# faustomorales/keras-ocr

Measured on AMD Instinct MI355X. Metric: images/sec end-to-end Pipeline.recognize() @768x768, higher is better.
Workload: dtype f32 (fp32 operands as 2 fp16 pieces [F(4,3) / head layers] or 3 bf16 pieces [1x1, dilated], 3 / 6 MFMA products, fp32 accumulate; fp32-class error vs fp64: tests/test_conv_gpu.py)

## Files before the change

### include/kocr.h

```cpp
#ifndef KOCR_H
#define KOCR_H

#include <stdint.h>

#ifdef __cplusplus
extern "C" {
#endif

typedef struct kocr_ctx kocr_ctx;

enum {
  KOCR_OK = 0,
  KOCR_EINVAL = -1,
  KOCR_EHIP = -2,
  KOCR_ENOWEIGHTS = -3,
  KOCR_ECAPACITY = -4,
  KOCR_ENOMEM = -5,
  KOCR_EEMPTYCONTOUR = -6,
  KOCR_EZERODIV = -7
};

enum { KOCR_U8 = 0, KOCR_F32 = 1 };

int kocr_create(kocr_ctx** out, int hip_device);
// ... 71 lines not shown
                     int64_t cap_lines, int64_t* true_lines, int flags);

int kocr_detect(kocr_ctx* ctx, const void* img, int dtype, int N, int H, int W,
                float detection_threshold, float text_threshold, float link_threshold,
                int size_threshold, int micro_batch, float* boxes, int32_t* counts, int cap,
                int on_device);

int kocr_recognize_boxes(kocr_ctx* ctx, const uint8_t* img_rgb, int N, int H, int W,
                         const float* boxes, const int32_t* counts, int32_t* labels, int on_device);

int kocr_resize_pad(kocr_ctx* ctx, const uint8_t* src, int n, int sh, int sw, int dh, int dw,
                    int Hmax, int Wmax, int cval, uint8_t* dst, int on_device);

int kocr_pipeline(kocr_ctx* ctx, int N, const uint8_t* const* imgs, const int32_t* hs,
                  const int32_t* ws, const int32_t* dhs, const int32_t* dws, int Hmax, int Wmax,
                  float detection_threshold, float text_threshold, float link_threshold,
                  int size_threshold, int micro_batch, float* boxes, int32_t* counts, int cap,
                  int32_t* labels, int max_crops, int32_t* n_crops, int on_device);

int kocr_pipeline_results(kocr_ctx* ctx, float* boxes, int cap, int32_t* labels, int max_crops);

int kocr_pipeline_device_results(kocr_ctx* ctx, const float** d_boxes, const int32_t** d_counts, const int32_t** d_labels,
                                 int32_t* N, int32_t* cap, int32_t* M);

int kocr_conv2d_nhwc(kocr_ctx* ctx, const float* in, int N, int H, int W, int Cin,
                     const float* w_hwio, int KH, int KW, int dilation, int Cout,
                     const float* pre_a, const float* pre_b, int relu,
                     const float* post_a, const float* post_b, float* out);

int kocr_conv2d_cells(kocr_ctx* ctx, const float* in, int N, int H, int W, int Cin, const float* w_hwio, int Cout,
                      const float* pre_a, const float* pre_b, int relu, const float* post_a, const float* post_b,
                      int cellW, int cellWv, int pool, float* out, float* pool_out, float* amax_out);

#define KOCR_SPLIT_BF16X3 0
#define KOCR_SPLIT_F16X2 1
#define KOCR_SPLIT_F16X1 2
int kocr_set_split_mode(kocr_ctx* ctx, int mode);
int kocr_get_split_mode(const kocr_ctx* ctx);

int kocr_set_schedule(kocr_ctx* ctx, int fold_linear_chain, int fold_upsample);
int kocr_get_schedule(kocr_ctx* ctx, int* fold_linear_chain, int* fold_upsample);

#define KOCR_RECT_EXACT 0
#define KOCR_RECT_OPENCV 1
int kocr_set_min_area_rect(kocr_ctx* ctx, int rule);
int kocr_get_min_area_rect(const kocr_ctx* ctx);

int kocr_set_scores(kocr_ctx* ctx, int on);
int kocr_get_scores(const kocr_ctx* ctx);
int kocr_detection_scores(kocr_ctx* ctx, float* scores, int cap);
int kocr_recognition_scores(kocr_ctx* ctx, float* log_word, float* char_scores, int max_crops, int32_t* n_crops,
                            int32_t* label_width);
int kocr_crnn_forward_scores(kocr_ctx* ctx, const float* crops, int M, int32_t* labels, float* probs, float* log_word,
                             float* char_scores, int on_device);

int kocr_crnn_beam(kocr_ctx* ctx, const float* crops, int M, int beam_width, int top_paths, int32_t* labels, float* log_prob,
                   int on_device);
int kocr_set_beam(kocr_ctx* ctx, int beam_width, int top_paths);
int kocr_get_beam(const kocr_ctx* ctx, int* beam_width, int* top_paths);
int kocr_recognition_beams(kocr_ctx* ctx, int32_t* labels, float* log_prob, int max_crops, int32_t* n_crops,
                           int32_t* label_width, int32_t* top_paths);

#define KOCR_LEXICON_MAX_WORD 32
int kocr_set_lexicon(kocr_ctx* ctx, const int32_t* words, int stride, const int32_t* lengths, int V);
int kocr_lexicon_size(const kocr_ctx* ctx);
int kocr_crnn_lexicon(kocr_ctx* ctx, const float* crops, int M, int top_words, int32_t* index, float* log_prob, float* all_values,
// ... 19 lines not shown
```

### keras_ocr_amd/_lib.py

```python
import contextlib
import ctypes
import math
import os

import numpy as np

_HERE = os.path.dirname(os.path.abspath(__file__))
LIB_PATH = os.path.join(_HERE, "csrc", "libkocr.so")

KOCR_U8, KOCR_F32 = 0, 1
KOCR_OK, KOCR_EINVAL, KOCR_EHIP, KOCR_ENOWEIGHTS, KOCR_ECAPACITY, KOCR_ENOMEM, KOCR_EEMPTYCONTOUR, KOCR_EZERODIV = range(0, -8, -1)
MIN_AREA_RECT_RULES = {"exact": 0, "opencv": 1}

_c_float_p = ctypes.POINTER(ctypes.c_float)
_c_int_p = ctypes.POINTER(ctypes.c_int)
_c_i64_p = ctypes.POINTER(ctypes.c_int64)
_c_dbl_p = ctypes.POINTER(ctypes.c_double)

_lib = None


class KocrError(RuntimeError):
    """A libkocr call returned a non-zero code."""

# ... 46 lines not shown
        "kocr_set_lexicon_scratch": (ci, [vp, ctypes.c_uint64]),
        "kocr_set_scores": (ci, [vp, ci]),
        "kocr_get_scores": (ci, [vp]),
        "kocr_detection_scores": (ci, [vp, vp, ci]),
        "kocr_recognition_scores": (ci, [vp, vp, vp, ci, vp, vp]),
        "kocr_crnn_classes": (ci, [vp]),
        "kocr_crnn_label_width": (ci, [vp]),
        "kocr_crnn_set_rnn_steps_to_discard": (ci, [vp, ci]),
        "kocr_ctc_batch_cost": (ci, [vp, vp, ci, ci, ci, vp, ci, vp, vp, vp, ci]),
        "kocr_crnn_ctc_loss": (ci, [vp, vp, ci, vp, ci, vp, vp, vp, ci]),
        "kocr_crnn_features": (ci, [vp, vp, ci, vp, ci]),
        "kocr_compute_maps": (ci, [vp, vp, ci, ci, ci, ci, ci, ci, vp, vp, ci, vp, vp, vp, ci]),
        "kocr_heat_mse": (ci, [vp, vp, vp, ci, ci, ci, vp, ci]),
        "kocr_craft_mse": (ci, [vp, vp, ci, ci, ci, ci, vp, ci, vp, ci]),
        "kocr_iou_table": (ci, [vp, ci, vp, vp, vp, vp, vp, ctypes.c_int64, vp, ci]),
        "kocr_score": (ci, [vp, ci, vp, vp, vp, vp, vp, vp, vp, vp, vp, ctypes.c_double, ctypes.c_double, vp, vp, vp, vp, vp,
                            ctypes.c_int64, vp, ci]),
        "kocr_group_lines": (ci, [vp, ci, vp, vp, ctypes.c_double, ctypes.c_double, ctypes.c_double, ctypes.c_double, vp, vp, vp, vp,
                                  ctypes.c_int64, vp, ci]),
        "kocr_get_boxes": (ci, [vp, vp, ci, ci, ci, ctypes.c_float, ctypes.c_float, ctypes.c_float, ci, vp, vp, ci, ci]),
        "kocr_warp_crops": (ci, [vp, vp, ci, ci, ci, vp, vp, ci, ci, vp, ci]),
        "kocr_warp_quads": (ci, [vp, vp, ci, ci, ci, ci, vp, vp, vp, vp, vp, ci, ci, vp, vp]),
        "kocr_detect": (ci, [vp, vp, ci, ci, ci, ci, ctypes.c_float, ctypes.c_float, ctypes.c_float, ci, ci, vp, vp, ci, ci]),
        "kocr_recognize_boxes": (ci, [vp, vp, ci, ci, ci, vp, vp, vp, ci]),
        "kocr_resize_pad": (ci, [vp, vp, ci, ci, ci, ci, ci, ci, ci, ci, vp, ci]),
        "kocr_pipeline": (ci, [vp, ci, ctypes.POINTER(vp), _c_int_p, _c_int_p, _c_int_p, _c_int_p, ci, ci,
                               ctypes.c_float, ctypes.c_float, ctypes.c_float, ci, ci, vp, vp, ci, vp, ci, vp, ci]),
        "kocr_pipeline_device_results": (ci, [vp, vp, vp, vp, vp, vp, vp]),
        "kocr_pipeline_results": (ci, [vp, vp, ci, vp, ci]),
        "kocr_resize_pad_f32": (ci, [vp, vp, ci, ci, ci, ci, ci, ci, ci, ci, ctypes.c_float, vp]),
        "kocr_warp_crops_f32": (ci, [vp, vp, ci, ci, ci, ci, vp, vp, ci, ci, vp]),
        "kocr_conv2d_nhwc": (ci, [vp, vp, ci, ci, ci, ci, vp, ci, ci, ci, ci, vp, vp, ci, vp, vp, vp]),
        "kocr_conv2d_cells": (ci, [vp, vp, ci, ci, ci, ci, vp, ci, vp, vp, ci, vp, vp, ci, ci, ci, vp, vp, vp]),
        "kocr_set_split_mode": (ci, [vp, ci]),
        "kocr_get_split_mode": (ci, [vp]),
        "kocr_set_schedule": (ci, [vp, ci, ci]),
        "kocr_get_schedule": (ci, [vp, _c_int_p, _c_int_p]),
        "kocr_set_min_area_rect": (ci, [vp, ci]),
        "kocr_get_min_area_rect": (ci, [vp]),
        "kocr_profile_enable": (ci, [vp, ci]),
        "kocr_profile_reset": (ci, [vp]),
        "kocr_profile_report": (ci, [vp, ci, ctypes.c_char_p, _c_i64_p, _c_dbl_p, _c_dbl_p, _c_dbl_p]),
        "kocr_range_stats_enable": (ci, [vp, ci]),
        "kocr_range_stats_report": (ci, [vp, ci, ctypes.c_char_p, _c_dbl_p]),
    }
    for name, (res, args) in sigs.items():
        if not hasattr(lib, name):
            continue
        fn = getattr(lib, name)
        fn.restype = res
        fn.argtypes = args
    _lib = lib
    return lib


def _ptr(a):
    if a is None:
        return ctypes.c_void_p(0)
    if isinstance(a, (int, np.integer)):
        return ctypes.c_void_p(int(a))
    return ctypes.c_void_p(a.ctypes.data)


def beam_args(beam_width, top_paths=1):
    bw, k = int(beam_width), int(top_paths)
    if not 1 <= bw <= 64:
# ... 534 lines not shown
        self._check(self._lib.kocr_pipeline_device_results(self._h, ctypes.byref(pb), ctypes.byref(pc), ctypes.byref(pl),
                                                           ctypes.byref(n), ctypes.byref(cap), ctypes.byref(m)))
        return {"boxes": pb.value or 0, "counts": pc.value or 0, "labels": pl.value or 0, "n": n.value, "cap": cap.value, "m": m.value}

    def conv2d_nhwc(self, x, w_hwio, dilation=1, pre_a=None, pre_b=None, relu=False, post_a=None, post_b=None):
        x = np.ascontiguousarray(x, dtype=np.float32)
        w = np.ascontiguousarray(w_hwio, dtype=np.float32)
        n, h, wd, cin = x.shape
        kh, kw, cin2, cout = w.shape
        assert cin == cin2
        out = np.empty((n, h, wd, cout), dtype=np.float32)
        vecs = [None if v is None else np.ascontiguousarray(v, dtype=np.float32) for v in (pre_a, pre_b, post_a, post_b)]
        self._check(self._lib.kocr_conv2d_nhwc(self._h, _ptr(x), n, h, wd, cin, _ptr(w), kh, kw, int(dilation), cout,
                                               _ptr(vecs[0]), _ptr(vecs[1]), int(bool(relu)), _ptr(vecs[2]),
                                               _ptr(vecs[3]), _ptr(out)))
        return out

    def conv2d_cells(self, x, w_hwio, cell_w, cell_wv, pool=False, need_full=True, pre_a=None, pre_b=None, relu=False,
                     post_a=None, post_b=None):
        x = np.ascontiguousarray(x, dtype=np.float32)
        w = np.ascontiguousarray(w_hwio, dtype=np.float32)
        n, h, wd, cin = x.shape
        assert w.shape[:3] == (3, 3, cin)
        cout = w.shape[3]
        out = np.empty((n, h, wd, cout), dtype=np.float32) if (need_full or not pool) else None
        pooled = np.empty((n, h // 2, wd // 2, cout), dtype=np.float32) if pool else None
        amax = np.zeros((n, wd // cell_w), dtype=np.float32)
        vecs = [None if v is None else np.ascontiguousarray(v, dtype=np.float32) for v in (pre_a, pre_b, post_a, post_b)]
        self._check(self._lib.kocr_conv2d_cells(self._h, _ptr(x), n, h, wd, cin, _ptr(w), cout, _ptr(vecs[0]), _ptr(vecs[1]),
                                                int(bool(relu)), _ptr(vecs[2]), _ptr(vecs[3]), int(cell_w), int(cell_wv),
                                                int(bool(pool)), _ptr(out), _ptr(pooled), _ptr(amax)))
        return out, pooled, amax

    SPLIT_BF16X3, SPLIT_F16X2, SPLIT_F16X1 = 0, 1, 2

    def set_split_mode(self, mode):
        if isinstance(mode, str):
            mode = {"bf16": 0, "bf16x3": 0, "f16": 1, "fp16": 1, "f16x2": 1, "f16x1": 2, "fast": 2}[mode]
        self._check(self._lib.kocr_set_split_mode(self._h, int(mode)))

    def get_split_mode(self):
        return self._check(self._lib.kocr_get_split_mode(self._h))

    def set_schedule(self, fold_linear_chain=True, fold_upsample=True):
        self._check(self._lib.kocr_set_schedule(self._h, int(bool(fold_linear_chain)), int(bool(fold_upsample))))

    def get_schedule(self):
        lin, up = ctypes.c_int(0), ctypes.c_int(0)
        self._check(self._lib.kocr_get_schedule(self._h, ctypes.byref(lin), ctypes.byref(up)))
        return bool(lin.value), bool(up.value)

    def set_min_area_rect(self, rule):
        self._check(self._lib.kocr_set_min_area_rect(self._h, _min_area_rect_code(rule)))

    def get_min_area_rect(self):
        code = self._check(self._lib.kocr_get_min_area_rect(self._h))
        return {v: k for k, v in MIN_AREA_RECT_RULES.items()}[code]

    @contextlib.contextmanager
    def _min_area_rect_scope(self, rule):
        if rule is None:
            yield
            return
        code = _min_area_rect_code(rule)
        old = self._check(self._lib.kocr_get_min_area_rect(self._h))
        self._check(self._lib.kocr_set_min_area_rect(self._h, code))
# ... 191 lines not shown
```

### keras_ocr_amd/csrc/api.cpp

```cpp
#include "abi.h"
#include "taps.h"
#include <cmath>
#include <algorithm>
#include <mutex>
#include <set>

int arena_reserve(kocr_ctx* ctx, Arena& a, size_t bytes) {
  ctx->last_pl.valid = false;
  ctx->last_sc.clear();
  ctx->last_beam.clear();
  ctx->last_lex.clear();
  if (bytes <= a.cap) return KOCR_OK;
  if (a.base) {
    KOCR_HIP(ctx, hipStreamSynchronize(ctx->stream));
    KOCR_HIP(ctx, hipFree(a.base));
    a.base = nullptr;
    a.cap = 0;
  }
  const size_t want = bytes + (bytes >> 3) + 4096;
  void* p = nullptr;
  hipError_t e = hipMalloc(&p, want);
  if (e != hipSuccess) {
    ctx->set_err("workspace hipMalloc(" + std::to_string(want) + " B) failed: " + hipGetErrorString(e));
    return KOCR_ENOMEM;
// ... 912 lines not shown
  ti.C = ti.cs = Cin;
  to.C = to.cs = tp.C = tp.cs = Cout;
  ti.cellW = to.cellW = cellW;
  ti.cellWv = to.cellWv = cellWv;
  tp.cellW = cellW / 2;
  tp.cellWv = cellWv / 2;
  ti.amax = ctx->amax_slots(N * cn);
  to.amax = ctx->amax_slots(N * cn);
  tp.amax = ctx->amax_slots(N * cn);
  if (!ti.amax || !to.amax || !tp.amax) KOCR_FAIL(ctx, KOCR_ECAPACITY, "kocr_conv2d_cells: out of max-|x| slots");
  const float* d_in;
  KOCR_TRY(st.in(in, nin, d_in));
  ti.p = (float*)d_in;
  if (out) KOCR_TRY(st.out(out, nout, to.p));
  if (pool) KOCR_TRY(st.out(pool_out, npool, tp.p));
  std::vector<float> am((size_t)N * cn, 0.f);
  for (int n = 0; n < N; ++n)
    for (int y = 0; y < H; ++y)
      for (int x = 0; x < W; ++x) {
        const float* px = in + (((size_t)n * H + y) * W + x) * Cin;
        float m = 0.f;
        for (int c = 0; c < Cin; ++c) m = std::max(m, std::fabs(px[c]));
        float& a = am[(size_t)n * cn + x / cellW];
        a = std::max(a, m);
      }
  KOCR_TRY(st.put((float*)ti.amax, am.data(), am.size() * sizeof(float)));
  KOCR_TRY(launch_conv_pool(ctx, L, ti, nullptr, nullptr, to, pool ? &tp : nullptr, out != nullptr));
  if (out) KOCR_TRY(st.back(out, to.p, nout));
  if (pool) KOCR_TRY(st.back(pool_out, tp.p, npool));
  if (amax_out) KOCR_TRY(st.download(amax_out, (const float*)(pool && !out ? tp.amax : to.amax), am.size() * sizeof(float)));
  return st.finish();
}

int kocr_set_split_mode(kocr_ctx* ctx, int mode) {
  if (!ctx) return KOCR_EINVAL;
  if (mode != KOCR_SPLIT_BF16X3 && mode != KOCR_SPLIT_F16X2 && mode != KOCR_SPLIT_F16X1) KOCR_FAIL(ctx, KOCR_EINVAL, "kocr_set_split_mode: unknown mode");
  ctx->split_mode = mode;
  return KOCR_OK;
}

int kocr_get_split_mode(const kocr_ctx* ctx) { return ctx ? ctx->split_mode : KOCR_EINVAL; }

int kocr_set_schedule(kocr_ctx* ctx, int fold_linear_chain, int fold_upsample) {
  if (!ctx) return KOCR_EINVAL;
  ctx->opt_linfold = fold_linear_chain != 0;
  ctx->opt_upfold = fold_upsample != 0;
  return KOCR_OK;
}

int kocr_get_schedule(kocr_ctx* ctx, int* fold_linear_chain, int* fold_upsample) {
  if (!ctx || !fold_linear_chain || !fold_upsample) return KOCR_EINVAL;
  *fold_linear_chain = ctx->opt_linfold ? 1 : 0;
  *fold_upsample = ctx->opt_upfold ? 1 : 0;
  return KOCR_OK;
}

int kocr_set_min_area_rect(kocr_ctx* ctx, int rule) {
  if (!ctx) return KOCR_EINVAL;
  if (rule != KOCR_RECT_EXACT && rule != KOCR_RECT_OPENCV) KOCR_FAIL(ctx, KOCR_EINVAL, "kocr_set_min_area_rect: unknown rule");
  ctx->min_area_rect = rule;
  return KOCR_OK;
}

int kocr_get_min_area_rect(const kocr_ctx* ctx) { return ctx ? ctx->min_area_rect : KOCR_EINVAL; }

int kocr_set_scores(kocr_ctx* ctx, int on) {
// ... 103 lines not shown
```

### keras_ocr_amd/csrc/conv_w43h.hip

```cpp
#include "w43_common.h"
#include "probe_clock.h"

namespace {

#define W4H_SCALED_CONSTANTS(sc)                                                                       \
  const float k_s = (sc), k_sA = (sc) * W4_A, k_sB = (sc) * W4_B, k_sA2 = (sc) * W4_A2, k_sB2 = (sc) * W4_B2, \
              k_sA2B2 = (sc) * W4_A2B2, k_sA2PB2 = (sc) * W4_A2PB2
template <class T>
__device__ __forceinline__ T w4h_transform(const T (&d)[6], int xi, float k_s, float k_sA, float k_sB, float k_sA2, float k_sB2,
                                           float k_sA2B2, float k_sA2PB2) {
  switch (xi) {
    case 0: return (k_sA2B2 * d[0] - k_sA2PB2 * d[2]) + k_s * d[4];
    case 1: return (k_s * d[4] - k_sB2 * d[2]) + k_sA * (d[3] - W4_B2 * d[1]);
    case 2: return (k_s * d[4] - k_sB2 * d[2]) - k_sA * (d[3] - W4_B2 * d[1]);
    case 3: return (k_s * d[4] - k_sA2 * d[2]) + k_sB * (d[3] - W4_A2 * d[1]);
    case 4: return (k_s * d[4] - k_sA2 * d[2]) - k_sB * (d[3] - W4_A2 * d[1]);
    default: return (k_sA2B2 * d[1] - k_sA2PB2 * d[3]) + k_s * d[5];
  }
}

constexpr int W4H_TOP = 12;

}

// ... 219 lines not shown
  const unsigned wlane = (unsigned)lane * 16u;
  auto w_tile = [&](int nt) { return (unsigned)__builtin_amdgcn_readfirstlane((nt * 4 + wn) * 12 * 64 * 16); };
  hf8 bw[2][6][NP];
  f16v acc[6][2];
  const int a_lane = GEO == 2 ? slot(l31 >> 3, l5, l31 & 7) : slot(l31 >> 4, l5, l31 & 15);
  const int a_lane1 = GEO == 2 ? slot((l31 >> 3) + 1, l5, l31 & 7) : 0;
  auto load_a = [&](hf8 (&a)[2][NP], const unsigned short* bufp, int ky, int xi) __attribute__((always_inline)) {
    if constexpr (DBG & 8) return;
    const unsigned short* plane = bufp + xi * NP * PLANE_R;
#pragma unroll
    for (int s = NP - 1; s >= 0; --s)
#pragma unroll
      for (int m = 0; m < 2; ++m) {
        int off;
        if constexpr (GEO == 2) {
          const int c = ky + 4 * m;
          off = ((c & 1) ? a_lane1 : a_lane) + (c >> 1) * 256;
        } else {
          off = a_lane + (ky + 2 * m) * ROW_STRIDE;
        }
        a[m][s] = *reinterpret_cast<const hf8*>(plane + s * PLANE_R + off);
      }
  };
  auto mfma_pt = [&](const hf8 (&a)[2][NP], const hf8 (&b)[NP], int xi) __attribute__((always_inline)) {
    if constexpr (DBG & 4) {
#pragma unroll
      for (int m = 0; m < 2; ++m)
#pragma unroll
        for (int s = 0; s < NP; ++s) acc[xi][m][s] += __builtin_bit_cast(v4f, a[m][s])[0] + __builtin_bit_cast(v4f, b[s])[0];
      return;
    }
    if constexpr (NP == 2) {
#pragma unroll
      for (int m = 0; m < 2; ++m) acc[xi][m] = __builtin_amdgcn_mfma_f32_32x32x16_f16(a[m][1], b[0], acc[xi][m], 0, 0, 0);
#pragma unroll
      for (int m = 0; m < 2; ++m) acc[xi][m] = __builtin_amdgcn_mfma_f32_32x32x16_f16(a[m][0], b[1], acc[xi][m], 0, 0, 0);
    }
#pragma unroll
    for (int m = 0; m < 2; ++m) acc[xi][m] = __builtin_amdgcn_mfma_f32_32x32x16_f16(a[m][0], b[0], acc[xi][m], 0, 0, 0);
  };
  hf8 a0[2][NP], a1[2][NP];
  auto step = [&](auto ky_c, auto slot_c, const unsigned short* bufc, unsigned short* bufn, unsigned w_next, float sc0, float sc1, int scq) __attribute__((always_inline)) {
    constexpr int KY = decltype(ky_c)::value;
    constexpr int SLOT = decltype(slot_c)::value;
    auto load_b = [&](int xi) __attribute__((always_inline)) {
      if constexpr (DBG & 2) return;
#pragma unroll
      for (int s = 0; s < NP; ++s)
        bw[SLOT][xi][s] = __builtin_bit_cast(hf8, __builtin_amdgcn_raw_buffer_load_b128(wrsrc, wlane, (int)(w_next + (unsigned)(xi * 2 + s) * 1024u), 0));
    };
    auto produce = [&](int xi) __attribute__((always_inline)) {
      if constexpr (KY == 0) produce4(raw0, bufn, xi, 0, sc0, sc1, scq);
      if constexpr (KY == 1) produce2(raw1, bufn, xi, sc0, sc1, scq);
    };
    auto interleave = [&]() __attribute__((always_inline)) {
      __builtin_amdgcn_sched_group_barrier(0x100, 2 * NP, 0);
      if constexpr (KY < 2) {
        constexpr int VPG = (KY == 0 ? 30 : 16) / (2 * PR - 1) + 1;
#pragma unroll
        for (int i = 0; i < 2 * PR - 1; ++i) {
          __builtin_amdgcn_sched_group_barrier(0x008, 1, 0);
          __builtin_amdgcn_sched_group_barrier(0x002, VPG, 0);
        }
        __builtin_amdgcn_sched_group_barrier(0x200, NP, 0);
        __builtin_amdgcn_sched_group_barrier(0x008, 1, 0);
      } else {
        __builtin_amdgcn_sched_group_barrier(0x008, 2 * PR, 0);
      }
    };
#pragma unroll
    for (int q = 0; q < 3; ++q) {
      __builtin_amdgcn_sched_barrier(0);
// ... 71 lines not shown
    for (int x = 0; x < 6; ++x)
#pragma unroll
      for (int m = 0; m < 2; ++m)
#pragma unroll
        for (int r = 0; r < 16; ++r) acc[x][m][r] = 0.f;
    PROBE_T(5);
    __builtin_amdgcn_s_waitcnt(0x0F70);
    PROBE_T(4);
    for (int cg = 0; cg < ncg; cg += 2) {
      using I0 = std::integral_constant<int, 0>;
      using I1 = std::integral_constant<int, 1>;
      using I2 = std::integral_constant<int, 2>;
      step(I0{}, I0{}, As, As + BUF_R, w_at(3 * cg + 2), s_cur, s_cur1, qb_cur);
      load_item0(raw0);
      step(I1{}, I1{}, As, As + BUF_R, w_at(3 * cg + 3), s_cur, s_cur1, qb_cur);
      load_item1(raw1);
      advance();
      step(I2{}, I0{}, As, As + BUF_R, w_at(3 * cg + 4), s_cur, s_cur1, qb_cur);
      const bool same = cg + 2 < ncg;
      const float s_odd = same ? s_cur : s_nxt, s_odd1 = same ? s_cur1 : s_nxt1;
      const int qb_odd = same ? qb_cur : qb_nxt;
      step(I0{}, I1{}, As + BUF_R, As, w_at(3 * cg + 5), s_odd, s_odd1, qb_odd);
      load_item0(raw0);
      step(I1{}, I0{}, As + BUF_R, As, w_at(3 * cg + 6), s_odd, s_odd1, qb_odd);
      load_item1(raw1);
      advance();
      step(I2{}, I1{}, As + BUF_R, As, w_at(3 * cg + 7), s_odd, s_odd1, qb_odd);
    }
    PROBE_T(0);

    {
      const int lane_e = kocr_fresh_lane();
      const int l31e = lane_e & 31, l5e = lane_e >> 5;
      const int n = (nt * 4 + wn) * 32 + l31e;
      int ty0, tx0, timg = 0;
      const long tpm = tile_org(mp, ty0, tx0, timg);
      int nimg, nimg1 = 0, cell0_x = 0;
      if constexpr (MODE == 2) {
        const int j0 = (int)w4_fdiv((unsigned)tx0, p.dv_wc);
        const int j1 = j0 + 1 < p.cells_per_row ? j0 + 1 : j0;
        nimg = __builtin_amdgcn_readfirstlane(timg * p.cells_per_row + j0);
        nimg1 = __builtin_amdgcn_readfirstlane(timg * p.cells_per_row + j1);
        cell0_x = j0 * p.cellW;
      } else if constexpr (MODE == 1) {
        nimg = __builtin_amdgcn_readfirstlane(timg);
      } else {
        nimg = __builtin_amdgcn_readfirstlane((int)w4_fdiv((unsigned)tpm, p.dv_hw));
      }
      const unsigned seen_out = p.amax_out ? kocr_amax_peek(p.amax_out + nimg) : 0u;
      const unsigned seen_pool = p.amax_pool ? kocr_amax_peek(p.amax_pool + nimg) : 0u;
      unsigned seen_out1 = 0u, seen_pool1 = 0u;
      if constexpr (MODE == 2) {
        seen_out1 = p.amax_out ? kocr_amax_peek(p.amax_out + nimg1) : 0u;
        seen_pool1 = p.amax_pool ? kocr_amax_peek(p.amax_pool + nimg1) : 0u;
      }
      const float pa = coef[n] * unscale, pb = coef[p.Cout_pad + n];
      const float pa1 = coef[n] * unscale1;
      const bool has_post = p.post_a != nullptr;
      const float qa = coef[2 * p.Cout_pad + n], qb = coef[3 * p.Cout_pad + n];
      const bool live = n < p.Cout;
      const float lo = p.relu ? 0.f : -INFINITY;
      auto act = [&](float v, float a) { return fmaxf(v * a + pb, lo); };
      const int l5q = 4 * l5e;
      auto qx_of = [&](int r) { return GEO == 2 ? (r & 3) + l5q : (r & 3) + 8 * ((r >> 2) & 1) + l5q; };
      auto first_row = [&](int m, int r) { return m == 0 && (GEO == 2 ? (r >> 2) == 0 : r < 8); };
#pragma unroll
      for (int m = 0; m < 2; ++m)
#pragma unroll
        for (int r = 0; r < 16; ++r) {
          float par = pa;
          if constexpr (MODE == 2) par = qx_of(r) < qb_cur ? pa : pa1;
          const float m0 = acc[0][m][r], m1 = acc[1][m][r], m2 = acc[2][m][r], m3 = acc[3][m][r], m4 = acc[4][m][r],
                      m5 = acc[5][m][r];
          const float s12 = m1 + m2, d12 = m1 - m2, s34 = m3 + m4, d34 = m3 - m4;
          acc[0][m][r] = act((m0 + s12) + s34, par);
          acc[1][m][r] = act(W4_A * d12 + W4_B * d34, par);
          acc[2][m][r] = act(W4_A2 * s12 + W4_B2 * s34, par);
          acc[3][m][r] = act((W4_A3 * d12 + W4_B3 * d34) + m5, par);
        }
      if (has_post) {
#pragma unroll
        for (int j = 0; j < 4; ++j)
#pragma unroll
          for (int m = 0; m < 2; ++m)
#pragma unroll
            for (int r = 0; r < 16; ++r) acc[j][m][r] = acc[j][m][r] * qa + qb;
      }
      if constexpr (MODE == 2) {
        const bool top = ty0 == 0;
#pragma unroll
        for (int r = 0; r < 16; ++r) {
          const int qx = qx_of(r);
          const int cx = tx0 + 4 * qx - (qx < qb_cur ? cell0_x : cell0_x + p.cellW);
#pragma unroll
          for (int j = 0; j < 4; ++j) {
            const bool v = cx + j < p.cellWv;
#pragma unroll
            for (int m = 0; m < 2; ++m) acc[j][m][r] = (v && !(top && first_row(m, r))) ? acc[j][m][r] : 0.f;
          }
        }
      }
      int ocs4 = p.out_cs * 4;
      asm volatile("" : "+s"(ocs4));
      int pcs4 = p.pool_cs * 4;
      asm volatile("" : "+s"(pcs4));
      if (p.amax_out || p.amax_pool) {
        if constexpr (MODE == 2) {
          float mx0 = 0.f, mx1 = 0.f;
#pragma unroll
          for (int r = 0; r < 16; ++r) {
            float mq = 0.f;
#pragma unroll
            for (int j = 0; j < 4; ++j)
#pragma unroll
              for (int m = 0; m < 2; ++m) mq = fmaxf(mq, fabsf(acc[j][m][r]));
            const bool first = qx_of(r) < qb_cur;
            mx0 = fmaxf(mx0, first ? mq : 0.f);
            mx1 = fmaxf(mx1, first ? 0.f : mq);
          }
          mx0 = live ? mx0 : 0.f;
          mx1 = live ? mx1 : 0.f;
          if (p.amax_out) kocr_amax_update_known(p.amax_out + nimg, mx0, seen_out);
          if (p.amax_pool) kocr_amax_update_known(p.amax_pool + nimg, mx0, seen_pool);
          if (qb_cur < QPR) {
            if (p.amax_out) kocr_amax_update_known(p.amax_out + nimg1, mx1, seen_out1);
            if (p.amax_pool) kocr_amax_update_known(p.amax_pool + nimg1, mx1, seen_pool1);
          }
        } else {
          float mx = 0.f;
#pragma unroll
          for (int j = 0; j < 4; ++j)
#pragma unroll
            for (int m = 0; m < 2; ++m)
#pragma unroll
              for (int r = 0; r < 16; ++r) mx = fmaxf(mx, fabsf(acc[j][m][r]));
          mx = live ? mx : 0.f;
          if (p.amax_out) kocr_amax_update_known(p.amax_out + nimg, mx, seen_out);
          if (p.amax_pool) kocr_amax_update_known(p.amax_pool + nimg, mx, seen_pool);
        }
      }
      PROBE_T(2);
      if constexpr (GEO == 2) {
        const __amdgpu_buffer_rsrc_t ro = w4_rsrc(p.out + (tpm * p.out_cs + p.out_co), 0x7FFFFFFFu);
        const unsigned vo = live ? (unsigned)((16 * l5e * p.out_cs + n) * 4) : OOB;
        const int wlim = p.W - tx0 - 16 * l5e;
#pragma unroll
        for (int m = 0; m < 2; ++m)
#pragma unroll
          for (int r = 0; r < 16; ++r) {
            const int px = (4 * m + (r >> 2)) * p.W + 4 * (r & 3);
            if (MODE == 1 && ty0 + 4 * m + (r >> 2) >= p.H) continue;
#pragma unroll
            for (int j = 0; j < 4; ++j) {
              const unsigned vom = MODE == 1 ? (4 * (r & 3) + j < wlim ? vo : OOB) : vo;
              __builtin_amdgcn_raw_buffer_store_b32(__float_as_uint(acc[j][m][r]), ro, vom, (px + j) * ocs4, 0);
            }
          }
      } else {
#pragma unroll
        for (int m = 0; m < 2; ++m) {
          const long pm = tpm + (long)2 * m * p.W;
          const int x0 = tx0;
          if (!POOL || p.write_full) {
            const __amdgpu_buffer_rsrc_t ro = w4_rsrc(p.out + (pm * p.out_cs + p.out_co), 0x7FFFFFFFu);
            const unsigned vo = live ? (unsigned)((16 * l5e * p.out_cs + n) * 4) : OOB;
            if constexpr (MODE == 1) {
              const int wlim = p.W - tx0 - 16 * l5e;
#pragma unroll
              for (int h = 0; h < 2; ++h) {
                if (ty0 + 2 * m + h >= p.H) continue;
#pragma unroll
                for (int r = 0; r < 8; ++r) {
                  const int px = 4 * ((r & 3) + 8 * (r >> 2));
#pragma unroll
                  for (int j = 0; j < 4; ++j)
                    __builtin_amdgcn_raw_buffer_store_b32(__float_as_uint(acc[j][m][r + 8 * h]), ro, px + j < wlim ? vo : OOB,
                                                          (px + j + h * p.W) * ocs4, 0);
                }
              }
            } else {
#pragma unroll
              for (int r = 0; r < 8; ++r) {
                const int px = 4 * ((r & 3) + 8 * (r >> 2));
#pragma unroll
                for (int j = 0; j < 4; ++j) {
                  __builtin_amdgcn_raw_buffer_store_b32(__float_as_uint(acc[j][m][r]), ro, vo, (px + j) * ocs4, 0);
                  __builtin_amdgcn_raw_buffer_store_b32(__float_as_uint(acc[j][m][r + 8]), ro, vo, (px + j + p.W) * ocs4, 0);
                }
              }
            }
          }
          if constexpr (POOL) {
            long pp0;
            if constexpr (MODE == 1)
              pp0 = ((long)timg * (p.H >> 1) + (ty0 >> 1) + m) * (p.W >> 1) + (x0 >> 1);
            else
              pp0 = ((pm - x0) >> 2) + (x0 >> 1);
            const __amdgpu_buffer_rsrc_t rp = w4_rsrc(p.pool_out + (pp0 * p.pool_cs + p.pool_co), 0x7FFFFFFFu);
            const unsigned vp = live ? (unsigned)((8 * l5e * p.pool_cs + n) * 4) : OOB;
            if (MODE == 1 && (ty0 >> 1) + m >= (p.H >> 1)) continue;
            const int plim = (p.W >> 1) - (x0 >> 1) - 8 * l5e;
            const bool ztop = MODE == 2 && ty0 == 0 && m == 0;
#pragma unroll
            for (int r = 0; r < 8; ++r) {
              const int pq = 2 * ((r & 3) + 8 * (r >> 2));
              float v0 = fmaxf(fmaxf(acc[0][m][r], acc[1][m][r]), fmaxf(acc[0][m][r + 8], acc[1][m][r + 8]));
              float v1 = fmaxf(fmaxf(acc[2][m][r], acc[3][m][r]), fmaxf(acc[2][m][r + 8], acc[3][m][r + 8]));
              if constexpr (MODE == 2) {
                v0 = ztop ? 0.f : v0;
                v1 = ztop ? 0.f : v1;
              }
              __builtin_amdgcn_raw_buffer_store_b32(__float_as_uint(v0), rp, (MODE != 1 || pq < plim) ? vp : OOB, pq * pcs4, 0);
              __builtin_amdgcn_raw_buffer_store_b32(__float_as_uint(v1), rp, (MODE != 1 || pq + 1 < plim) ? vp : OOB, (pq + 1) * pcs4, 0);
            }
          }
        }
      }
      PROBE_T(3);
    }
    gc = gn;
    lc = ln;
    rc = rn;
    make_geo(L + 2 * G, gn, ln, rn);
    ld_next = false;
    PROBE_T(1);
  }
  PROBE_TEND(tid == 0, 0, 6);
}

template <int POOL, int NP, int MODE = 0, int OCC = 1>
__global__ __launch_bounds__(256, OCC) void conv_w43rh_kernel(W4Params p) {
  static_assert(MODE == 0 || MODE == 1, "exact tiling or ragged");
  constexpr int NBW = 3;
  constexpr int PR = NP == 2 ? 3 : 1;
  constexpr int NROWS = 6, QPR = 16, KHS = QPR * 8, ROW_STRIDE = 2 * KHS, PLANE_R = NROWS * ROW_STRIDE;
  constexpr int BUF_R = 6 * NP * PLANE_R;
  constexpr int TCOLS = QPR * 4;
  extern __shared__ __attribute__((aligned(16))) unsigned short As[];
  float* coef = reinterpret_cast<float*>(OCC == 2 ? As + 2 * BUF_R : As + BUF_R + 4 * 16 * 64 * 8);
  const int tid = threadIdx.x, lane = tid & 63;
  const int wave = __builtin_amdgcn_readfirstlane(tid >> 6);
  const int wn = wave & 1, ph = wave >> 1;
  const int l31 = lane & 31, l5 = lane >> 5;
  const int total = p.total_tiles;
  const int ncg = p.Cin >> 4;
  const int G = gridDim.x;
  constexpr unsigned OOB = 0x80000000u;

  auto tile_mt = [&](int mp, int m) {
    const int rq = (int)w4_fdiv((unsigned)mp, p.dv_tpr), cb = mp - rq * p.tiles_per_row;
// ... 937 lines not shown
```

### keras_ocr_amd/csrc/split_common.h

```cpp
#pragma once
#include "common.h"
#include <cstring>

typedef short bf8 __attribute__((ext_vector_type(8)));
typedef _Float16 hf8 __attribute__((ext_vector_type(8)));
typedef _Float16 hf2 __attribute__((ext_vector_type(2)));
typedef float f16v __attribute__((ext_vector_type(16)));
typedef float v4f __attribute__((ext_vector_type(4)));
typedef unsigned u2v __attribute__((ext_vector_type(2)));
typedef float v2f __attribute__((ext_vector_type(2)));

__device__ __forceinline__ int kocr_xcd_remap(int bid, int nwg) {
  const int xcd = bid & 7;
  const int q = nwg >> 3, r = nwg & 7;
  return (xcd < r ? xcd * (q + 1) : r * (q + 1) + (xcd - r) * q) + (bid >> 3);
}

__device__ __forceinline__ void kocr_split4(const v4f v, u2v& h, u2v& m, u2v& l) {
  unsigned uh[4], um[4], ul[4];
#pragma unroll
  for (int c = 0; c < 4; ++c) {
    uh[c] = __float_as_uint(v[c]) & 0xFFFF0000u;
    const float r = v[c] - __uint_as_float(uh[c]);
    um[c] = __float_as_uint(r) & 0xFFFF0000u;
    ul[c] = __float_as_uint(r - __uint_as_float(um[c]));
  }
  h = u2v{__builtin_amdgcn_perm(uh[1], uh[0], 0x07060302u), __builtin_amdgcn_perm(uh[3], uh[2], 0x07060302u)};
  m = u2v{__builtin_amdgcn_perm(um[1], um[0], 0x07060302u), __builtin_amdgcn_perm(um[3], um[2], 0x07060302u)};
  l = u2v{__builtin_amdgcn_perm(ul[1], ul[0], 0x07060302u), __builtin_amdgcn_perm(ul[3], ul[2], 0x07060302u)};
}

__device__ __forceinline__ void kocr_split2(const v2f v, unsigned& h, unsigned& m, unsigned& l) {
  unsigned uh[2], um[2], ul[2];
#pragma unroll
  for (int c = 0; c < 2; ++c) {
    uh[c] = __float_as_uint(v[c]) & 0xFFFF0000u;
    const float r = v[c] - __uint_as_float(uh[c]);
    um[c] = __float_as_uint(r) & 0xFFFF0000u;
    ul[c] = __float_as_uint(r - __uint_as_float(um[c]));
  }
  h = __builtin_amdgcn_perm(uh[1], uh[0], 0x07060302u);
  m = __builtin_amdgcn_perm(um[1], um[0], 0x07060302u);
// ... 61 lines not shown
```

### keras_ocr_amd/scores.py

```python
import collections
import math

import numpy as np

Score = collections.namedtuple("Score", ["detection", "word", "log_word", "characters"])
Score.__doc__ = """One word's scores.

detection: the maximum of the detector's text map over the box's connected component (float; ``None`` where no detector
    ran, as in ``Recognizer.recognize``).
word: ``exp(log_word)``, the probability the recogniser gives the returned text.
log_word: the log of the summed probability of every CTC alignment that collapses to the returned text (float).
characters: float32 array, one value per decoded label: the peak probability of that label over the frames that emitted it.
"""


def assemble(labels, log_word, char_scores, detection=None):
    lengths = (np.asarray(labels) >= 0).sum(axis=1) if len(labels) else []
    out = []
    for i, n in enumerate(lengths):
        lw = float(log_word[i])
        out.append(Score(None if detection is None else float(detection[i]), math.exp(lw), lw,
                         np.array(char_scores[i, :n], dtype=np.float32)))
    return out


def need(stage, obj, method):
    import inspect

    fn = getattr(obj, method)
    try:
        params = inspect.signature(fn).parameters
    except (TypeError, ValueError):
        params = {}
    if "return_scores" not in params:
        raise TypeError(f"return_scores=True: the {stage} ({type(obj).__name__}.{method}) cannot give scores "
                        "(it takes no return_scores argument)")
    return fn
```

Measured before the change: 260.5.

## Transpose Winograd conv MFMA operands so epilogue stores channel-contiguous 128-bit vectors

Swaps the A/B operands of the F(4,3) MFMA products so each lane holds four consecutive output channels instead of one channel across pixels. The epilogue is rebuilt around this: coefficients load as float4, pooling pairs rows with a permlane16 swap, and outputs go out as 128-bit buffer stores when channel counts and alignment allow, with a scalar fallback otherwise. The aim is to cut the many scattered 32-bit stores and per-row coefficient work in the output phase. It also adds a conv2d_view test entry point and a small change in scores.py. The risk lies in the new lane-to-pixel mapping and the masking and amax logic that depend on it.

```diff
diff --git a/include/kocr.h b/include/kocr.h
--- a/include/kocr.h
+++ b/include/kocr.h
@@ -127,6 +127,12 @@
                       const float* pre_a, const float* pre_b, int relu, const float* post_a, const float* post_b,
                       int cellW, int cellWv, int pool, float* out, float* pool_out, float* amax_out);
 
+int kocr_conv2d_view(kocr_ctx* ctx, const float* in, int N, int H, int W, int Cin, const float* w_hwio, int Cout,
+                     const float* pre_a, const float* pre_b, int relu, const float* post_a, const float* post_b,
+                     float* out_buf, int out_floats, int out_shift, int out_cs, int out_co,
+                     float* pool_buf, int pool_floats, int pool_shift, int pool_cs, int pool_co,
+                     float* amax_out, float* amax_pool);
+
 #define KOCR_SPLIT_BF16X3 0
 #define KOCR_SPLIT_F16X2 1
 #define KOCR_SPLIT_F16X1 2
diff --git a/keras_ocr_amd/_lib.py b/keras_ocr_amd/_lib.py
--- a/keras_ocr_amd/_lib.py
+++ b/keras_ocr_amd/_lib.py
@@ -102,6 +102,7 @@
         "kocr_warp_crops_f32": (ci, [vp, vp, ci, ci, ci, ci, vp, vp, ci, ci, vp]),
         "kocr_conv2d_nhwc": (ci, [vp, vp, ci, ci, ci, ci, vp, ci, ci, ci, ci, vp, vp, ci, vp, vp, vp]),
         "kocr_conv2d_cells": (ci, [vp, vp, ci, ci, ci, ci, vp, ci, vp, vp, ci, vp, vp, ci, ci, ci, vp, vp, vp]),
+        "kocr_conv2d_view": (ci, [vp, vp, ci, ci, ci, ci, vp, ci, vp, vp, ci, vp, vp, vp, ci, ci, ci, ci, vp, ci, ci, ci, ci, vp, vp]),
         "kocr_set_split_mode": (ci, [vp, ci]),
         "kocr_get_split_mode": (ci, [vp]),
         "kocr_set_schedule": (ci, [vp, ci, ci]),
@@ -702,6 +703,24 @@
                                                 int(bool(pool)), _ptr(out), _ptr(pooled), _ptr(amax)))
         return out, pooled, amax
 
+    def conv2d_view(self, x, w_hwio, out_buf=None, out_shift=0, out_cs=0, out_co=0, pool_buf=None, pool_shift=0, pool_cs=0,
+                    pool_co=0, pre_a=None, pre_b=None, relu=False, post_a=None, post_b=None):
+        x = np.ascontiguousarray(x, dtype=np.float32)
+        w = np.ascontiguousarray(w_hwio, dtype=np.float32)
+        n, h, wd, cin = x.shape
+        assert w.shape[:3] == (3, 3, cin)
+        for b in (out_buf, pool_buf):
+            assert b is None or (b.dtype == np.float32 and b.ndim == 1 and b.flags.c_contiguous and b.flags.writeable)
+        am_o = np.zeros(n, np.float32) if out_buf is not None else None
+        am_p = np.zeros(n, np.float32) if pool_buf is not None else None
+        vecs = [None if v is None else np.ascontiguousarray(v, dtype=np.float32) for v in (pre_a, pre_b, post_a, post_b)]
+        self._check(self._lib.kocr_conv2d_view(
+            self._h, _ptr(x), n, h, wd, cin, _ptr(w), w.shape[3], _ptr(vecs[0]), _ptr(vecs[1]), int(bool(relu)), _ptr(vecs[2]),
+            _ptr(vecs[3]), _ptr(out_buf), 0 if out_buf is None else out_buf.size, int(out_shift), int(out_cs), int(out_co),
+            _ptr(pool_buf), 0 if pool_buf is None else pool_buf.size, int(pool_shift), int(pool_cs), int(pool_co),
+            _ptr(am_o), _ptr(am_p)))
+        return am_o, am_p
+
     SPLIT_BF16X3, SPLIT_F16X2, SPLIT_F16X1 = 0, 1, 2
 
     def set_split_mode(self, mode):
diff --git a/keras_ocr_amd/csrc/api.cpp b/keras_ocr_amd/csrc/api.cpp
--- a/keras_ocr_amd/csrc/api.cpp
+++ b/keras_ocr_amd/csrc/api.cpp
@@ -968,6 +968,70 @@
   return st.finish();
 }
 
+int kocr_conv2d_view(kocr_ctx* ctx, const float* in, int N, int H, int W, int Cin, const float* w_hwio, int Cout,
+                     const float* pre_a, const float* pre_b, int relu, const float* post_a, const float* post_b,
+                     float* out_buf, int out_floats, int out_shift, int out_cs, int out_co,
+                     float* pool_buf, int pool_floats, int pool_shift, int pool_cs, int pool_co,
+                     float* amax_out, float* amax_pool) {
+  if (!ctx || !in || !w_hwio || (!out_buf && !pool_buf)) return KOCR_EINVAL;
+  if (N <= 0 || H <= 0 || W <= 0 || Cin <= 0 || Cout <= 0) KOCR_FAIL(ctx, KOCR_EINVAL, "kocr_conv2d_view: bad shape");
+  const size_t opx = (size_t)N * H * W, ppx = (size_t)N * (H / 2) * (W / 2);
+  if (out_buf && (out_shift < 0 || out_co < 0 || out_co + Cout > out_cs || (size_t)out_shift + opx * out_cs > (size_t)out_floats))
+    KOCR_FAIL(ctx, KOCR_EINVAL, "kocr_conv2d_view: the destination view does not fit its buffer");
+  if (pool_buf && (H < 2 || W < 2 || pool_shift < 0 || pool_co < 0 || pool_co + Cout > pool_cs ||
+                   (size_t)pool_shift + ppx * pool_cs > (size_t)pool_floats))
+    KOCR_FAIL(ctx, KOCR_EINVAL, "kocr_conv2d_view: the pooled view does not fit its buffer");
+  KOCR_HIP(ctx, hipSetDevice(ctx->device));
+  KOCR_TRY(ctx->amax_begin());
+  TempLayer layer(ctx);
+  ConvLayer L;
+  L.name = "kocr_conv2d_view";
+  KOCR_TRY(prepare_conv(ctx, L, w_hwio, false, Cin, Cout, 3, 3, 1, pre_a, pre_b, relu, post_a, post_b));
+  const size_t nin = opx * Cin * sizeof(float);
+  const size_t nout = out_buf ? (size_t)out_floats * sizeof(float) : 0, npool = pool_buf ? (size_t)pool_floats * sizeof(float) : 0;
+  Staging st{ctx, ctx->ws, "kocr_conv2d_view"};
+  const size_t nfull = out_buf ? 0 : opx * Cout * sizeof(float);
+  KOCR_TRY(st.reserve(0, {nin, nout, npool, nfull}));
+  Tensor ti, to, tp;
+  ti.N = to.N = tp.N = N;
+  ti.H = to.H = H;
+  ti.W = to.W = W;
+  tp.H = H / 2;
+  tp.W = W / 2;
+  ti.C = ti.cs = Cin;
+  to.C = tp.C = Cout;
+  to.cs = out_buf ? out_cs : Cout;
+  to.co = out_buf ? out_co : 0;
+  tp.cs = pool_cs;
+  tp.co = pool_co;
+  to.amax = ctx->amax_slots(N);
+  tp.amax = ctx->amax_slots(N);
+  if (!to.amax || !tp.amax) KOCR_FAIL(ctx, KOCR_ECAPACITY, "kocr_conv2d_view: out of max-|x| slots");
+  const float* d_in;
+  KOCR_TRY(st.in(in, nin, d_in));
+  ti.p = (float*)d_in;
+  float *d_out = nullptr, *d_pool = nullptr;
+  if (out_buf) {
+    const float* d;
+    KOCR_TRY(st.upload(out_buf, nout, d));
+    d_out = (float*)d;
+    to.p = d_out + out_shift;
+  }
+  if (!out_buf) KOCR_TRY(st.scratch(nfull, to.p));
+  if (pool_buf) {
+    const float* d;
+    KOCR_TRY(st.upload(pool_buf, npool, d));
+    d_pool = (float*)d;
+    tp.p = d_pool + pool_shift;
+  }
+  KOCR_TRY(launch_conv_pool(ctx, L, ti, nullptr, nullptr, to, pool_buf ? &tp : nullptr, out_buf != nullptr));
+  if (out_buf) KOCR_TRY(st.download(out_buf, (const float*)d_out, nout));
+  if (pool_buf) KOCR_TRY(st.download(pool_buf, (const float*)d_pool, npool));
+  if (amax_out && out_buf) KOCR_TRY(st.download(amax_out, (const float*)to.amax, (size_t)N * sizeof(float)));
+  if (amax_pool && pool_buf) KOCR_TRY(st.download(amax_pool, (const float*)tp.amax, (size_t)N * sizeof(float)));
+  return st.finish();
+}
+
 int kocr_set_split_mode(kocr_ctx* ctx, int mode) {
   if (!ctx) return KOCR_EINVAL;
   if (mode != KOCR_SPLIT_BF16X3 && mode != KOCR_SPLIT_F16X2 && mode != KOCR_SPLIT_F16X1) KOCR_FAIL(ctx, KOCR_EINVAL, "kocr_set_split_mode: unknown mode");
diff --git a/keras_ocr_amd/csrc/conv_w43h.hip b/keras_ocr_amd/csrc/conv_w43h.hip
--- a/keras_ocr_amd/csrc/conv_w43h.hip
+++ b/keras_ocr_amd/csrc/conv_w43h.hip
@@ -275,12 +275,12 @@
     }
     if constexpr (NP == 2) {
 #pragma unroll
-      for (int m = 0; m < 2; ++m) acc[xi][m] = __builtin_amdgcn_mfma_f32_32x32x16_f16(a[m][1], b[0], acc[xi][m], 0, 0, 0);
-#pragma unroll
-      for (int m = 0; m < 2; ++m) acc[xi][m] = __builtin_amdgcn_mfma_f32_32x32x16_f16(a[m][0], b[1], acc[xi][m], 0, 0, 0);
-    }
-#pragma unroll
-    for (int m = 0; m < 2; ++m) acc[xi][m] = __builtin_amdgcn_mfma_f32_32x32x16_f16(a[m][0], b[0], acc[xi][m], 0, 0, 0);
+      for (int m = 0; m < 2; ++m) acc[xi][m] = __builtin_amdgcn_mfma_f32_32x32x16_f16(b[0], a[m][1], acc[xi][m], 0, 0, 0);
+#pragma unroll
+      for (int m = 0; m < 2; ++m) acc[xi][m] = __builtin_amdgcn_mfma_f32_32x32x16_f16(b[1], a[m][0], acc[xi][m], 0, 0, 0);
+    }
+#pragma unroll
+    for (int m = 0; m < 2; ++m) acc[xi][m] = __builtin_amdgcn_mfma_f32_32x32x16_f16(b[0], a[m][0], acc[xi][m], 0, 0, 0);
   };
   hf8 a0[2][NP], a1[2][NP];
   auto step = [&](auto ky_c, auto slot_c, const unsigned short* bufc, unsigned short* bufn, unsigned w_next, float sc0, float sc1, int scq) __attribute__((always_inline)) {
@@ -418,7 +418,9 @@
     {
       const int lane_e = kocr_fresh_lane();
       const int l31e = lane_e & 31, l5e = lane_e >> 5;
-      const int n = (nt * 4 + wn) * 32 + l31e;
+      const int rr = GEO == 2 ? l31e >> 3 : l31e >> 4, qx = GEO == 2 ? l31e & 7 : l31e & 15;
+      constexpr int RPM = GEO == 2 ? 4 : 2;
+      const int n0 = (nt * 4 + wn) * 32 + 4 * l5e;
       int ty0, tx0, timg = 0;
       const long tpm = tile_org(mp, ty0, tx0, timg);
       int nimg, nimg1 = 0, cell0_x = 0;
@@ -440,72 +442,76 @@
         seen_out1 = p.amax_out ? kocr_amax_peek(p.amax_out + nimg1) : 0u;
         seen_pool1 = p.amax_pool ? kocr_amax_peek(p.amax_pool + nimg1) : 0u;
       }
-      const float pa = coef[n] * unscale, pb = coef[p.Cout_pad + n];
-      const float pa1 = coef[n] * unscale1;
+      const bool cell0 = MODE != 2 || qx < qb_cur;
+      const float uns = cell0 ? unscale : unscale1;
       const bool has_post = p.post_a != nullptr;
-      const float qa = coef[2 * p.Cout_pad + n], qb = coef[3 * p.Cout_pad + n];
-      const bool live = n < p.Cout;
       const float lo = p.relu ? 0.f : -INFINITY;
-      auto act = [&](float v, float a) { return fmaxf(v * a + pb, lo); };
-      const int l5q = 4 * l5e;
-      auto qx_of = [&](int r) { return GEO == 2 ? (r & 3) + l5q : (r & 3) + 8 * ((r >> 2) & 1) + l5q; };
-      auto first_row = [&](int m, int r) { return m == 0 && (GEO == 2 ? (r >> 2) == 0 : r < 8); };
-#pragma unroll
-      for (int m = 0; m < 2; ++m)
-#pragma unroll
-        for (int r = 0; r < 16; ++r) {
-          float par = pa;
-          if constexpr (MODE == 2) par = qx_of(r) < qb_cur ? pa : pa1;
-          const float m0 = acc[0][m][r], m1 = acc[1][m][r], m2 = acc[2][m][r], m3 = acc[3][m][r], m4 = acc[4][m][r],
-                      m5 = acc[5][m][r];
-          const float s12 = m1 + m2, d12 = m1 - m2, s34 = m3 + m4, d34 = m3 - m4;
-          acc[0][m][r] = act((m0 + s12) + s34, par);
-          acc[1][m][r] = act(W4_A * d12 + W4_B * d34, par);
-          acc[2][m][r] = act(W4_A2 * s12 + W4_B2 * s34, par);
-          acc[3][m][r] = act((W4_A3 * d12 + W4_B3 * d34) + m5, par);
-        }
+      const float* cf = coef + n0;
+      v4f ca_n = *reinterpret_cast<const v4f*>(cf), cb_n = *reinterpret_cast<const v4f*>(cf + p.Cout_pad);
+#pragma unroll
+      for (int g = 0; g < 4; ++g) {
+        const v4f pa = ca_n * uns, pb = cb_n;
+        if (g < 3) {
+          ca_n = *reinterpret_cast<const v4f*>(cf + 8 * (g + 1));
+          cb_n = *reinterpret_cast<const v4f*>(cf + p.Cout_pad + 8 * (g + 1));
+        }
+        __builtin_amdgcn_sched_barrier(0);
+#pragma unroll
+        for (int m = 0; m < 2; ++m)
+#pragma unroll
+          for (int i = 0; i < 4; ++i) {
+            const int r = 4 * g + i;
+            const float par = pa[i], pbr = pb[i];
+            auto act = [&](float v) { return fmaxf(v * par + pbr, lo); };
+            const float m0 = acc[0][m][r], m1 = acc[1][m][r], m2 = acc[2][m][r], m3 = acc[3][m][r], m4 = acc[4][m][r],
+                        m5 = acc[5][m][r];
+            const float s12 = m1 + m2, d12 = m1 - m2, s34 = m3 + m4, d34 = m3 - m4;
+            acc[0][m][r] = act((m0 + s12) + s34);
+            acc[1][m][r] = act(W4_A * d12 + W4_B * d34);
+            acc[2][m][r] = act(W4_A2 * s12 + W4_B2 * s34);
+            acc[3][m][r] = act((W4_A3 * d12 + W4_B3 * d34) + m5);
+          }
+      }
       if (has_post) {
 #pragma unroll
+        for (int g = 0; g < 4; ++g) {
+          __builtin_amdgcn_sched_barrier(0);
+          const v4f qa = *reinterpret_cast<const v4f*>(cf + 2 * p.Cout_pad + 8 * g);
+          const v4f qb = *reinterpret_cast<const v4f*>(cf + 3 * p.Cout_pad + 8 * g);
+#pragma unroll
+          for (int j = 0; j < 4; ++j)
+#pragma unroll
+            for (int m = 0; m < 2; ++m)
+#pragma unroll
+              for (int i = 0; i < 4; ++i) acc[j][m][4 * g + i] = acc[j][m][4 * g + i] * qa[i] + qb[i];
+        }
+      }
+      if constexpr (MODE == 2) {
+        const int cx = tx0 + 4 * qx - (cell0 ? cell0_x : cell0_x + p.cellW);
+#pragma unroll
         for (int j = 0; j < 4; ++j)
 #pragma unroll
-          for (int m = 0; m < 2; ++m)
-#pragma unroll
-            for (int r = 0; r < 16; ++r) acc[j][m][r] = acc[j][m][r] * qa + qb;
-      }
-      if constexpr (MODE == 2) {
-        const bool top = ty0 == 0;
-#pragma unroll
-        for (int r = 0; r < 16; ++r) {
-          const int qx = qx_of(r);
-          const int cx = tx0 + 4 * qx - (qx < qb_cur ? cell0_x : cell0_x + p.cellW);
-#pragma unroll
-          for (int j = 0; j < 4; ++j) {
-            const bool v = cx + j < p.cellWv;
-#pragma unroll
-            for (int m = 0; m < 2; ++m) acc[j][m][r] = (v && !(top && first_row(m, r))) ? acc[j][m][r] : 0.f;
+          for (int m = 0; m < 2; ++m) {
+            const bool keep = cx + j < p.cellWv && !(m == 0 && ty0 == 0 && rr == 0);
+#pragma unroll
+            for (int r = 0; r < 16; ++r) acc[j][m][r] = keep ? acc[j][m][r] : 0.f;
           }
-        }
       }
       int ocs4 = p.out_cs * 4;
       asm volatile("" : "+s"(ocs4));
-      int pcs4 = p.pool_cs * 4;
-      asm volatile("" : "+s"(pcs4));
       if (p.amax_out || p.amax_pool) {
+        float mx = 0.f;
+#pragma unroll
+        for (int r = 0; r < 16; ++r) {
+          float mq = 0.f;
+#pragma unroll
+          for (int j = 0; j < 4; ++j)
+#pragma unroll
+            for (int m = 0; m < 2; ++m) mq = fmaxf(mq, fabsf(acc[j][m][r]));
+          mx = fmaxf(mx, n0 + 8 * (r >> 2) + (r & 3) < p.Cout ? mq : 0.f);
+        }
         if constexpr (MODE == 2) {
-          float mx0 = 0.f, mx1 = 0.f;
-#pragma unroll
-          for (int r = 0; r < 16; ++r) {
-            float mq = 0.f;
-#pragma unroll
-            for (int j = 0; j < 4; ++j)
-#pragma unroll
-              for (int m = 0; m < 2; ++m) mq = fmaxf(mq, fabsf(acc[j][m][r]));
-            const bool first = qx_of(r) < qb_cur;
-            mx0 = fmaxf(mx0, first ? mq : 0.f);
-            mx1 = fmaxf(mx1, first ? 0.f : mq);
-          }
-          mx0 = live ? mx0 : 0.f;
-          mx1 = live ? mx1 : 0.f;
+          const float mx0 = cell0 ? mx : 0.f, mx1 = cell0 ? 0.f : mx;
           if (p.amax_out) kocr_amax_update_known(p.amax_out + nimg, mx0, seen_out);
           if (p.amax_pool) kocr_amax_update_known(p.amax_pool + nimg, mx0, seen_pool);
           if (qb_cur < QPR) {
@@ -513,95 +519,77 @@
             if (p.amax_pool) kocr_amax_update_known(p.amax_pool + nimg1, mx1, seen_pool1);
           }
         } else {
-          float mx = 0.f;
-#pragma unroll
-          for (int j = 0; j < 4; ++j)
-#pragma unroll
-            for (int m = 0; m < 2; ++m)
-#pragma unroll
-              for (int r = 0; r < 16; ++r) mx = fmaxf(mx, fabsf(acc[j][m][r]));
-          mx = live ? mx : 0.f;
           if (p.amax_out) kocr_amax_update_known(p.amax_out + nimg, mx, seen_out);
           if (p.amax_pool) kocr_amax_update_known(p.amax_pool + nimg, mx, seen_pool);
         }
       }
       PROBE_T(2);
-      if constexpr (GEO == 2) {
-        const __amdgpu_buffer_rsrc_t ro = w4_rsrc(p.out + (tpm * p.out_cs + p.out_co), 0x7FFFFFFFu);
-        const unsigned vo = live ? (unsigned)((16 * l5e * p.out_cs + n) * 4) : OOB;
-        const int wlim = p.W - tx0 - 16 * l5e;
-#pragma unroll
-        for (int m = 0; m < 2; ++m)
-#pragma unroll
-          for (int r = 0; r < 16; ++r) {
-            const int px = (4 * m + (r >> 2)) * p.W + 4 * (r & 3);
-            if (MODE == 1 && ty0 + 4 * m + (r >> 2) >= p.H) continue;
+      const bool full = !POOL || p.write_full;
+      const bool vec_ok = (p.Cout & 3) == 0 &&
+                          (!full || (((p.out_cs | p.out_co) & 3) == 0 && ((unsigned long long)p.out & 15) == 0)) &&
+                          (!POOL || (((p.pool_cs | p.pool_co) & 3) == 0 && ((unsigned long long)p.pool_out & 15) == 0));
+      auto emit = [&](auto v16_c) __attribute__((always_inline)) {
+        constexpr bool V16 = decltype(v16_c)::value;
+        auto put = [&](const __amdgpu_buffer_rsrc_t rs, const v4f x, unsigned vpx, int soff, int g) __attribute__((always_inline)) {
+          if constexpr (V16) {
+            __builtin_amdgcn_raw_buffer_store_b128(__builtin_bit_cast(u4v, x), rs, n0 + 8 * g < p.Cout ? vpx : OOB, soff + 32 * g, 0);
+          } else {
+#pragma unroll
+            for (int i = 0; i < 4; ++i)
+              __builtin_amdgcn_raw_buffer_store_b32(__float_as_uint(x[i]), rs, n0 + 8 * g + i < p.Cout ? vpx : OOB, soff + 32 * g + 4 * i, 0);
+          }
+        };
+#pragma unroll
+        for (int m = 0; m < 2; ++m) {
+          if (full) {
+            const long pm = tpm + (long)RPM * m * p.W;
+            const __amdgpu_buffer_rsrc_t ro = w4_rsrc(p.out + (pm * p.out_cs + p.out_co), 0x7FFFFFFFu);
+            const unsigned vo = (unsigned)(((rr * p.W + 4 * qx) * p.out_cs + n0) * 4);
+            const bool row_ok = MODE != 1 || ty0 + RPM * m + rr < p.H;
+            const int wlim = p.W - tx0 - 4 * qx;
 #pragma unroll
             for (int j = 0; j < 4; ++j) {
-              const unsigned vom = MODE == 1 ? (4 * (r & 3) + j < wlim ? vo : OOB) : vo;
-              __builtin_amdgcn_raw_buffer_store_b32(__float_as_uint(acc[j][m][r]), ro, vom, (px + j) * ocs4, 0);
-            }
-          }
-      } else {
-#pragma unroll
-        for (int m = 0; m < 2; ++m) {
-          const long pm = tpm + (long)2 * m * p.W;
-          const int x0 = tx0;
-          if (!POOL || p.write_full) {
-            const __amdgpu_buffer_rsrc_t ro = w4_rsrc(p.out + (pm * p.out_cs + p.out_co), 0x7FFFFFFFu);
-            const unsigned vo = live ? (unsigned)((16 * l5e * p.out_cs + n) * 4) : OOB;
-            if constexpr (MODE == 1) {
-              const int wlim = p.W - tx0 - 16 * l5e;
-#pragma unroll
-              for (int h = 0; h < 2; ++h) {
-                if (ty0 + 2 * m + h >= p.H) continue;
-#pragma unroll
-                for (int r = 0; r < 8; ++r) {
-                  const int px = 4 * ((r & 3) + 8 * (r >> 2));
-#pragma unroll
-                  for (int j = 0; j < 4; ++j)
-                    __builtin_amdgcn_raw_buffer_store_b32(__float_as_uint(acc[j][m][r + 8 * h]), ro, px + j < wlim ? vo : OOB,
-                                                          (px + j + h * p.W) * ocs4, 0);
-                }
-              }
-            } else {
-#pragma unroll
-              for (int r = 0; r < 8; ++r) {
-                const int px = 4 * ((r & 3) + 8 * (r >> 2));
-#pragma unroll
-                for (int j = 0; j < 4; ++j) {
-                  __builtin_amdgcn_raw_buffer_store_b32(__float_as_uint(acc[j][m][r]), ro, vo, (px + j) * ocs4, 0);
-                  __builtin_amdgcn_raw_buffer_store_b32(__float_as_uint(acc[j][m][r + 8]), ro, vo, (px + j + p.W) * ocs4, 0);
-                }
-              }
+              const unsigned vj = (row_ok && (MODE != 1 || j < wlim)) ? vo : OOB;
+#pragma unroll
+              for (int g = 0; g < 4; ++g)
+                put(ro, v4f{acc[j][m][4 * g], acc[j][m][4 * g + 1], acc[j][m][4 * g + 2], acc[j][m][4 * g + 3]}, vj, j * ocs4, g);
             }
           }
           if constexpr (POOL) {
+            int pcs4 = p.pool_cs * 4;
+            asm volatile("" : "+s"(pcs4));
             long pp0;
             if constexpr (MODE == 1)
-              pp0 = ((long)timg * (p.H >> 1) + (ty0 >> 1) + m) * (p.W >> 1) + (x0 >> 1);
+              pp0 = ((long)timg * (p.H >> 1) + (ty0 >> 1) + m) * (p.W >> 1) + (tx0 >> 1);
             else
-              pp0 = ((pm - x0) >> 2) + (x0 >> 1);
+              pp0 = ((tpm + (long)2 * m * p.W - tx0) >> 2) + (tx0 >> 1);
             const __amdgpu_buffer_rsrc_t rp = w4_rsrc(p.pool_out + (pp0 * p.pool_cs + p.pool_co), 0x7FFFFFFFu);
-            const unsigned vp = live ? (unsigned)((8 * l5e * p.pool_cs + n) * 4) : OOB;
             if (MODE == 1 && (ty0 >> 1) + m >= (p.H >> 1)) continue;
-            const int plim = (p.W >> 1) - (x0 >> 1) - 8 * l5e;
+            const int pq = 2 * qx + rr;
+            const int plim = (p.W >> 1) - (tx0 >> 1);
+            const unsigned vp = (MODE != 1 || pq < plim) ? (unsigned)(pq * pcs4 + n0 * 4) : OOB;
             const bool ztop = MODE == 2 && ty0 == 0 && m == 0;
 #pragma unroll
-            for (int r = 0; r < 8; ++r) {
-              const int pq = 2 * ((r & 3) + 8 * (r >> 2));
-              float v0 = fmaxf(fmaxf(acc[0][m][r], acc[1][m][r]), fmaxf(acc[0][m][r + 8], acc[1][m][r + 8]));
-              float v1 = fmaxf(fmaxf(acc[2][m][r], acc[3][m][r]), fmaxf(acc[2][m][r + 8], acc[3][m][r + 8]));
-              if constexpr (MODE == 2) {
-                v0 = ztop ? 0.f : v0;
-                v1 = ztop ? 0.f : v1;
+            for (int g = 0; g < 4; ++g) {
+              __builtin_amdgcn_sched_barrier(0);
+              v4f v;
+#pragma unroll
+              for (int i = 0; i < 4; ++i) {
+                const int r = 4 * g + i;
+                const float a = fmaxf(acc[0][m][r], acc[1][m][r]), b = fmaxf(acc[2][m][r], acc[3][m][r]);
+                const u2v sw = __builtin_bit_cast(u2v, __builtin_amdgcn_permlane16_swap(__float_as_uint(a), __float_as_uint(b), false, false));
+                const float t = fmaxf(__uint_as_float(sw[0]), __uint_as_float(sw[1]));
+                v[i] = ztop ? 0.f : t;
               }
-              __builtin_amdgcn_raw_buffer_store_b32(__float_as_uint(v0), rp, (MODE != 1 || pq < plim) ? vp : OOB, pq * pcs4, 0);
-              __builtin_amdgcn_raw_buffer_store_b32(__float_as_uint(v1), rp, (MODE != 1 || pq + 1 < plim) ? vp : OOB, (pq + 1) * pcs4, 0);
+              put(rp, v, vp, 0, g);
             }
           }
         }
-      }
+      };
+      if (vec_ok)
+        emit(std::true_type{});
+      else
+        emit(std::false_type{});
       PROBE_T(3);
     }
     gc = gn;
diff --git a/keras_ocr_amd/csrc/split_common.h b/keras_ocr_amd/csrc/split_common.h
--- a/keras_ocr_amd/csrc/split_common.h
+++ b/keras_ocr_amd/csrc/split_common.h
@@ -8,6 +8,7 @@
 typedef float f16v __attribute__((ext_vector_type(16)));
 typedef float v4f __attribute__((ext_vector_type(4)));
 typedef unsigned u2v __attribute__((ext_vector_type(2)));
+typedef unsigned u4v __attribute__((ext_vector_type(4)));
 typedef float v2f __attribute__((ext_vector_type(2)));
 
 __device__ __forceinline__ int kocr_xcd_remap(int bid, int nwg) {
diff --git a/keras_ocr_amd/scores.py b/keras_ocr_amd/scores.py
--- a/keras_ocr_amd/scores.py
+++ b/keras_ocr_amd/scores.py
@@ -1,5 +1,4 @@
 import collections
-import math
 
 import numpy as np
 
@@ -19,7 +18,7 @@
     out = []
     for i, n in enumerate(lengths):
         lw = float(log_word[i])
-        out.append(Score(None if detection is None else float(detection[i]), math.exp(lw), lw,
+        out.append(Score(None if detection is None else float(detection[i]), float(np.exp(lw)), lw,
                          np.array(char_scores[i, :n], dtype=np.float32)))
     return out
 
```

Result: faster. 267.2 (median of 6 runs) (+2.6%).
